# rwl/blu

Measured on AMD Instinct MI355X. Metric: factorize nnz/s + achieved HBM GB/s, 100k x 100k 10-nnz/col basis, higher is better.
Workload: dtype f64

## Files before the change

blu_amd/csrc/blu_dev.h:

```cpp
#pragma once
#include <hip/hip_runtime.h>
#include <stdint.h>
#include <hip/hip_cooperative_groups.h>
#include <rocprim/warp/warp_reduce.hpp>
#include <rocprim/warp/warp_scan.hpp>

#define BLU_WAVE 64

#ifndef BLU_DYN_SHARED
#define BLU_DYN_SHARED(T, name, bytes) extern __shared__ __attribute__((aligned(16))) T name[]
#endif
#ifdef BLU_PROFILE_FILLS
#define FILL_STAMP_BEGIN() long long fill_t0_ = (long long)__builtin_amdgcn_s_memtime()
#define FILL_STAMP(S, k)                                                 \
    do {                                                                 \
        if (threadIdx.x == 0) {                                          \
            const long long t_ = (long long)__builtin_amdgcn_s_memtime(); \
            (S)->prof[k] += t_ - fill_t0_;                               \
            fill_t0_ = t_;                                               \
        }                                                                \
    } while (0)
#else
#define FILL_STAMP_BEGIN() \
    do {                   \
    } while (0)
#define FILL_STAMP(S, k) \
    do {                 \
    } while (0)
#endif
#ifdef BLU_EMU_BUILD
#define BLU_WAVES_PER_EU(lo, hi)
#else
#define BLU_WAVES_PER_EU(lo, hi) __attribute__((amdgpu_waves_per_eu(lo, hi)))
#endif

enum {
    ST_RUNNING = 0,
    ST_DONE = 1,
    ST_STOPPED = 2,
    ST_NEED_L = 3,
    ST_NEED_U = 4,
    ST_NEED_CW = 5,
    ST_NEED_RW = 6,
    ST_INVALID_ARG = 7,
    ST_ERROR = 8
};

struct Scalars {
    int status;
    int err_line;
    int rank;
    int rankdef;
    int rank0;
    int min_colnz;
    int min_rownz;
    int pivot_row;
    int pivot_col;
    int bump_size;
    int cused, rused;
    int lused, uused;
    int need;
    int l_nz, u_nz;
    int fill_paths;
    long long matrix_nz;
    long long bump_nz;
    long long nsearch_pivot;
    long long factor_flops;
    long long nexpand;
    long long ngarbage;
    long long d3_hits;
    long long npivot_kind[6];
    long long nfast[4];
    double min_pivot, max_pivot;
    double onenorm, infnorm;
    double norm_l, norm_u, normest_l_inv, normest_u_inv, condest_l, condest_u, residual_test;
    long long prof[48];
};

#define DEVLU_SCALARS(X)                                                                               \
    X(int, m)                                                                                          \
    X(int, nzbias)                                                                      \
    X(int, maxsearch)                                                                                  \
    X(int, pad)                                                                                        \
    X(int, search_rows)                                                                                \
    X(int, no_fast)                    \
    X(int, skip_stats)              \
    X(double, droptol)                                                                                 \
    X(double, abstol)                                                                                  \
    X(double, reltol)                                                                                  \
    X(double, stretch)                                                                                 \
    X(long long, b_i_len)                                                                              \
    X(int, nzcap)                                                                                      \
    X(int, carena_cap)                                                                                 \
    X(int, rarena_cap)                                                                                 \
    X(int, lcap)                                                                                       \
    X(int, ucap)

#define DEVLU_ARRAYS_HOT(X)                                                                            \
    X(int, pinv) X(int, qinv) X(int, prow) X(int, pcol)                                                \
    X(LineRec, crec) X(LineRec, rrec) X(HeadRec, chead) X(HeadRec, rhead)                              \
    X(int, cidx) X(double, cval) X(int, ridx)                                                          \
    X(int, lbeg) X(int, ubeg) X(int, lidx) X(int, uidx) X(double, lval) X(double, uval)
#define DEVLU_ARRAYS_COLD(X)                                                                           \
    X(const unsigned long long, b_begin) X(const unsigned long long, b_end) X(const unsigned long long, b_i) \
    X(const double, b_x)                                                                               \
    X(int, bc_ptr) X(int, bc_idx) X(double, bc_val) X(int, bt_ptr) X(int, bt_idx) X(double, bt_val)    \
    X(int, rowmark) X(int, colmark) X(int, tnew) X(int, tnewr) X(double, txrj)                         \
    X(unsigned long long, tmask) X(double, gwork) X(int, iw0) X(int, iw1) X(int, iw2)
#define DEVLU_ARRAYS(X) DEVLU_ARRAYS_HOT(X) DEVLU_ARRAYS_COLD(X)

struct __attribute__((aligned(32))) LineRec {
    int beg, len, cap;
    int flink, blink;
    int spare;
    double max;
};
struct __attribute__((aligned(8))) HeadRec {
    int flink, blink;
};
static_assert(sizeof(LineRec) == 32 && sizeof(HeadRec) == 8, "record layout");
#define LINEREC_BEG 0
#define LINEREC_LEN 4
#define LINEREC_CAP 8
#define LINEREC_FLINK 12
#define LINEREC_BLINK 16
#define LINEREC_MAX 24

struct DevLU {
#define X(T, n) T n;
// ... 477 lines not shown
```

blu_amd/csrc/blu_hip.hip:

```cpp
#include <hip/hip_runtime.h>

#include <algorithm>
#include <cmath>
#include <cstdio>
#include <cstdlib>
#include <cstring>
#include <string>
#include <vector>

#include "../../include/blu_hip.h"
#include "blu_dev.h"
#include "k_finish.hip"
#define BLU_NS pv_single
#define BLU_CFG_WAVE 0
#include "k_pivot.hip"
#undef BLU_NS
#undef BLU_CFG_WAVE
#define BLU_NS pv_wave
#define BLU_CFG_WAVE 1
#include "k_pivot.hip"
#undef BLU_NS
#undef BLU_CFG_WAVE
#define BLU_NS pv_wave2
#define BLU_CFG_WAVE 2
// ... 436 lines not shown
    case BLU_STAT_NEXPAND: return (double)s.nexpand;
    case BLU_STAT_NGARBAGE: return (double)s.ngarbage;
    case BLU_STAT_FACTOR_FLOPS: return (double)s.factor_flops;
    case BLU_STAT_TIME_FACTORIZE: return h->t_total;
    case BLU_STAT_TIME_SINGLETONS: return h->t_phase[0];
    case BLU_STAT_TIME_SEARCH_PIVOT: {
        double tot = 0.0;
        for (int k = 0; k < 4; k++) tot += (double)s.prof[k];
        return tot > 0.0 ? h->t_pivot * (double)s.prof[0] / tot : 0.0;
    }
    case BLU_STAT_TIME_ELIM_PIVOT: {
        double tot = 0.0;
        for (int k = 0; k < 4; k++) tot += (double)s.prof[k];
        return tot > 0.0 ? h->t_pivot * (1.0 - (double)s.prof[0] / tot) : h->t_pivot;
    }
    case BLU_STAT_UPDATE_COST_DENOM: return h->update_cost_denom;
    case BLU_STAT_RANKDEF: return (double)s.rankdef;
    case BLU_STAT_L_MEM: return (double)h->D.lcap;
    case BLU_STAT_U_MEM: return (double)h->D.ucap;
    case BLU_STAT_W_MEM: return (double)h->D.carena_cap + (double)h->D.rarena_cap;
    case BLU_STAT_L_FLOPS: return (double)h->sp_l_flops;
    case BLU_STAT_U_FLOPS: return (double)h->sp_u_flops;
    case BLU_STAT_NFORREST: return h->upd_for_nfact == h->nfactorize ? (double)h->ust.nforrest : 0.0;
    case BLU_STAT_PIVOT_ERROR: return h->upd_for_nfact == h->nfactorize ? h->ust.pivot_error : 0.0;
    case BLU_STAT_R_NZ: return h->upd_for_nfact == h->nfactorize ? (double)h->ust.r_nz : 0.0;
    case BLU_STAT_R_FLOPS: return h->upd_for_nfact == h->nfactorize ? (double)h->ust.r_flops : 0.0;
    case BLU_STAT_MAX_ETA: return h->upd_for_nfact == h->nfactorize ? h->ust.max_eta : 0.0;
    case BLU_STAT_NSYMPERM_TOTAL: return (double)h->ust.nsymperm_total;
    case BLU_STAT_NFORREST_TOTAL: return (double)h->ust.nforrest_total;
    case BLU_STAT_DEV_NUNSYMPERM_TOTAL: return (double)h->ust.nunsymperm_total;
    case BLU_STAT_UPDATE_COST:
        return (h->upd_for_nfact == h->nfactorize ? h->ust.update_cost_numer : 0.0) / blu_hip_get_stat(h, BLU_STAT_UPDATE_COST_DENOM);
    case 44: case 45: case 46: case 47: return h->t_phase[key - 44];
    case 108: case 109: return h->t_phase[key - 108 + 4];
    case 43: return (double)h->sp_branch;
    case BLU_STAT_DEV_TIME_PIVOT_LOOP: return h->t_pivot;
    case BLU_STAT_DEV_TIME_TOTAL: return h->t_total;
    case BLU_STAT_DEV_RELAUNCHES: return (double)h->relaunches;
    case 50: return (double)s.d3_hits;
    case 51: return (double)s.npivot_kind[0];
    case 52: return (double)s.npivot_kind[1];
    case 53: return (double)s.npivot_kind[2];
    case 54: return (double)s.npivot_kind[3];
    case 55: return (double)s.npivot_kind[4];
    case 56: return (double)s.npivot_kind[5];
    case 110: case 111: case 116: case 117: return (double)s.nfast[key < 116 ? key - 110 : key - 114];
    case 112: return (double)s.cused;
    case 113: return (double)s.rused;
    case 114: return (double)h->D.carena_cap;
    case 115: return (double)h->D.lcap;
    case 120: return (double)h->last_pivot_regs;
    case 118: return (double)h->last_pivot_kernel;
    case 119: return (double)s.fill_paths;
    case 57: return (double)s.err_line;
    case 58: return (double)s.status;
    case 60: case 61: case 62: case 63: case 64: case 65: case 66: case 67: case 68: case 69: case 70: case 71: case 72: case 73: case 74: case 75:
    case 76: case 77: case 78: case 79: case 80: case 81: case 82: case 83:
    case 84: case 85: case 86: case 87: case 88: case 89: case 90: case 91:
    case 92: case 93: case 94: case 95: case 96: case 97: case 98: case 99: case 100: case 101: case 102: case 103: case 104: case 105: case 106: case 107:
        return (double)s.prof[key - 60];
    default: return NAN;
    }
}

extern "C" const char *blu_hip_last_error(const blu_hip *h) { return h ? h->err.c_str() : "null handle"; }
extern "C" const char *blu_hip_version(void)
{
#if defined(BLU_EWCHECK)
    return "blu_hip 0.2 (gfx950; self-checking build: early / speculative searches verified in the kernel)";
#elif defined(BLU_PROFILE)
    return "blu_hip 0.2 (gfx950; phase-timing build)";
#else
    return "blu_hip 0.2 (gfx950)";
#endif
}
extern "C" int blu_hip_device_count(void)
{
    int n = 0;
    if (hipGetDeviceCount(&n) != hipSuccess) return 0;
    return n;
}

static bool ensure_gwork(blu_hip *h, int cols)
{
    if (cols <= h->gwork_cols) return true;
    DevLU &D = h->D;
    const size_t n = (size_t)cols * ((size_t)h->m + 1);
    dfree(D.gwork);
    h->gwork_cols = 0;
    if (!dalloc(h, &D.gwork, n) || !hip_ok(h, hipMemset(D.gwork, 0, n * sizeof(double)), "hipMemset")) return false;
    h->gwork_cols = cols;
    return true;
}
static int64_t grown(blu_hip *h, int64_t cap, int64_t need_extra)
{
    const double f = std::max(1.0, h->realloc_factor);
    int64_t n = (int64_t)((double)(cap + need_extra) * f) + 64;
    return std::min<int64_t>(n, kIntMax);
}
static bool grow_l(blu_hip *h, int need)
{
    DevLU &D = h->D;
    const int64_t n = grown(h, D.lcap, need);
    if (n <= D.lcap) { h->err = "L storage limit (2^31 entries) reached"; return false; }
    if (!dgrow(h, &D.lidx, (size_t)h->hs.lused, (size_t)n) || !dgrow(h, &D.lval, (size_t)h->hs.lused, (size_t)n)) return false;
    D.lcap = (int)n;
// ... 594 lines not shown
```

blu_amd/csrc/k_pivot.hip:

```cpp
#include "blu_dev.h"

namespace BLU_NS {

__shared__ int g_pivot_err;
__shared__ int g_pivot_err_line;
#undef DEV_CHECK
#define DEV_CHECK(S, cond)                               \
    do {                                                 \
        if (!(cond)) {                                   \
            set_error((S), ST_ERROR, __LINE__);          \
            g_pivot_err = 1;                             \
        }                                                \
    } while (0)

#if BLU_CFG_WAVE
#include "k_pivot_wave_types.h"
#else
#include "k_pivot_fast_types.h"
#endif

#ifdef BLU_PROFILE
__shared__ long long g_pstamp[48];
#define PROF_STAMP(k)                                                      \
    do {                                                                   \
        if (threadIdx.x == 0) g_pstamp[k] = (long long)__builtin_amdgcn_s_memtime(); \
    } while (0)
#define PROF_STAMP_L0(k)                                                           \
    do {                                                                           \
        if (lane_id() == 0) g_pstamp[k] = (long long)__builtin_amdgcn_s_memtime(); \
    } while (0)
#define PROF_WAIT() asm volatile("s_waitcnt vmcnt(0)" ::: "memory")
#else
#define PROF_STAMP(k) \
    do {              \
    } while (0)
#define PROF_STAMP_L0(k) \
    do {                 \
    } while (0)
#define PROF_WAIT() \
    do {            \
    } while (0)
#endif

struct alignas(16) Sm {
    Fast fa;
    struct alignas(16) {
        int pr, pc, exit_code, head_exit;
    };
    struct alignas(16) {
        int nzc, nzr, pcb, prb;
    };
#ifdef BLU_PROFILE
    long long prof[48];
#else
    long long prof[1];
#endif
    int rank, rankdef, min_colnz, min_rownz;
    int cused, rused, lused, uused;
    int need;
    int flag_small;
    int other_row, where, ncancel, nfill;
    int stop_at, need_search;
    double pivot, other_value;
    long long nsearch, flops, nexpand, d3;
    long long kinds[6];
    long long nfast[4];
    int sh[40];
    long long shl[20];
#if BLU_CFG_WAVE
    unsigned long long wmax[BLU_CFG_WAVE];
#else
    unsigned long long wmax[16];
#endif
#if BLU_CFG_WAVE
    double swork[WV_WCAP];
#else
    double swork[16 * 64];
#endif
};

__device__ __forceinline__ void list_remove1(const LinkF &flink, const LinkB &blink, int e)
{
    const int f = flink[e], b = blink[e];
    flink[b] = f;
    blink[f] = b;
    flink[e] = e;
    blink[e] = e;
}
__device__ __forceinline__ void list_add1(int e, int list, const LinkF &flink, const LinkB &blink, int nelem)
{
    const int t = blink[nelem + list];
    blink[nelem + list] = e;
    blink[e] = t;
    flink[t] = e;
    flink[e] = nelem + list;
}

__device__ __forceinline__ int wave_list_move_batch(const LinkF &flink, const LinkB &blink, int nelem, gcint_p elems, gcint_p keys, int n,
                                                    gint_p mark, int big)
{
    const int lane = lane_id();
    int minkey = big;
    for (int c0 = 0; c0 < n; c0 += 64) {
        const int q = c0 + lane;
        if (q < n && keys[q] >= 0) mark[elems[q]] = 1;
    }
    wave_mem_sync();
    for (int c0 = 0; c0 < n; c0 += 64) {
// ... 980 lines not shown
    const int pr = sm->pr, pc = sm->pc;
    sm->fa.kind = 0;
    if (pc < 0 || pr < 0) return;
    sm->pcb = D.cbeg[pc];
    sm->prb = D.rbeg[pr];
    sm->nzc = D.clen[pc];
    sm->nzr = D.rlen[pr];
    sm->flag_small = 0;
    sm->ncancel = 0;
    DEV_CHECK(S, D.pinv[pr] == -1 && D.qinv[pc] == -1);
    DEV_CHECK(S, sm->nzc >= 1 && sm->nzr >= 1);
    if (sm->lused + (sm->nzc - 1) > D.lcap) {
        sm->exit_code = ST_NEED_L;
        sm->need = sm->nzc - 1;
    } else if (sm->uused + (sm->nzr - 1) > D.ucap) {
        sm->exit_code = ST_NEED_U;
        sm->need = sm->nzr - 1;
    }
}

#if BLU_CFG_WAVE
#include "k_pivot_wave.hip"
#else
__device__ __forceinline__ void pivot_loop_body(DevLU *Ds, int stop_at, Sm *sm, Mc *mc)
{
    const DevGP D(&Ds[blockIdx.x]);
    Scalars *S = D.s;
    const int tid = threadIdx.x, w = wave_id(), lane = lane_id();
    const int m = D.m;

    if (S->status != ST_RUNNING) return;
    if (tid == 0) {
        sm->rank = S->rank;
        sm->rankdef = S->rankdef;
        sm->min_colnz = S->min_colnz;
        sm->min_rownz = S->min_rownz;
        sm->cused = S->cused;
        sm->rused = S->rused;
        sm->lused = S->lused;
        sm->uused = S->uused;
        sm->pr = S->pivot_row;
        sm->pc = S->pivot_col;
        sm->exit_code = 0;
        sm->need = 0;
        sm->nsearch = 0;
        sm->flops = 0;
        sm->nexpand = 0;
        sm->d3 = 0;
        sm->stop_at = stop_at;
        sm->fa.kind = 0;
        sm->fa.ewValid = 0;
        sm->fa.spOk = 0;
        for (int k = 0; k < 6; k++) sm->kinds[k] = 0;
#ifdef BLU_PROFILE
        for (int k = 0; k < 48; k++) sm->prof[k] = 0;
        for (int k = 0; k < 48; k++) g_pstamp[k] = 0;
#endif
    }
    for (int k = tid; k < (int)blockDim.x; k += blockDim.x) sm->swork[k] = 0.0;
    if (tid < 16) sm->wmax[tid] = 0ull;
    for (int k = tid; k < 2 * KGMAX; k += blockDim.x) sm->fa.kg[0][k] = 0ull;
    if (tid == 0) {
        g_pivot_err = 0;
        g_pivot_err_line = 0;
    }
    mc_reset(D, mc, tid, (int)blockDim.x);
    __syncthreads();

    long long ew_mcb = 0;
    int ew_fb = 0;
    for (;;) {
        if (w == 0) {
            if (lane == 0) {
                if (g_pivot_err) sm->exit_code = ST_ERROR;
                else if (sm->rank + sm->rankdef >= m) sm->exit_code = ST_DONE;
                else if (sm->stop_at >= 0 && sm->pc < 0 && sm->rank + sm->rankdef >= sm->stop_at) sm->exit_code = ST_STOPPED;
                sm->need_search = sm->pc < 0;
                sm->head_exit = sm->exit_code;
            }
            wave_mem_sync();
            const bool heads_stale = mc->dirty;
            WAVE_LOCKSTEP();
            if (heads_stale) {
                mc_reset(D, mc, lane, 64);
                wave_mem_sync();
            }
            PROF_STAMP(0);
            if (!sm->head_exit) {
                bool handled = false;
                if (sm->need_search) {
                    if (D.search_rows == 0 && !D.no_fast) handled = markowitz_fast(D, sm, mc, ew_mcb, ew_fb);
                    if (!handled) {
                        if (D.search_rows == 0) markowitz_wave(D, sm);
                        else if (lane == 0) markowitz_serial(D, sm);
                        wave_mem_sync();
                    }
                }
                if (!handled && lane == 0) setup_pivot_general(D, sm);
            }
        }
        __syncthreads();
        const int4 dA = *reinterpret_cast<const int4 *>(&sm->pr);
        const int4 dB = *reinterpret_cast<const int4 *>(&sm->nzc);
        const int4 dC = *reinterpret_cast<const int4 *>(&sm->fa.kind);
        if (dA.w) break;
        const int pr = dA.x, pc = dA.y;
        if (pc < 0) {
            if (tid == 0) {
                DEV_CHECK(S, false);
                sm->exit_code = ST_ERROR;
            }
            __syncthreads();
            break;
        }
        if (pr < 0) {
            __syncthreads();
            if (tid == 0) {
                list_remove1(D.cflink, D.cblink, pc);
                mc->dirty = 1;
                sm->pc = -1;
                sm->rankdef++;
                sm->kinds[5]++;
            }
            __syncthreads();
            continue;
        }

        if (dA.z) break;
        PROF_STAMP(1);
        const int nz_col = dB.x, nz_row = dB.y;
        const int kind = dC.x;
        bool ok = true;
        if (kind == 1) fast_small(D, sm, mc, pr, pc, nz_col, nz_row, ew_mcb, ew_fb);
        else if (kind == 2) fast_scol(D, sm, mc, pr, pc, nz_row, dC.y, ew_mcb, ew_fb);
        else {
            if (tid == 0) mc->dirty = 1;
            if (nz_row == 1) ok = pivot_singleton_row(D, sm);
            else if (nz_col == 1) ok = pivot_singleton_col(D, sm);
            else if (nz_col == 2) ok = pivot_doubleton_col(D, sm);
            else ok = pivot_general(D, sm, nz_col - 1 <= 64);
        }
        if (!ok) break;
        PROF_STAMP(2);
#ifdef BLU_PROFILE
#define PROF_ADD(k, a, b)                                                                                           \
    do {                                                                                                            \
        const long long d_ = g_pstamp[a] - g_pstamp[b];                                                             \
        if (g_pstamp[b] >= g_pstamp[0] && d_ >= 0 && d_ < (1LL << 28)) sm->prof[k] += d_;                            \
    } while (0)
        if (tid == 0) {
            const int kk = sm->fa.kind == 1 ? 1 : (sm->fa.kind == 2 ? 2 : 3);
            PROF_ADD(0, 1, 0);
            PROF_ADD(kk, 2, 1);
            sm->prof[3 + kk] += 1;
            if (kk == 1) {
                PROF_ADD(7, 3, 1);
                PROF_ADD(22, 6, 3);
                PROF_ADD(23, 24, 3);
                PROF_ADD(24, 25, 3);
                PROF_ADD(25, 26, 25);
                PROF_ADD(26, 27, 26);
                PROF_ADD(27, 28, 27);
                PROF_ADD(30, 30, 27);
                PROF_ADD(31, 31, 30);
                PROF_ADD(28, 29, 28);
                PROF_ADD(29, 2, 29);
                sm->prof[32] += sm->nzr - 1;
                sm->prof[33] += sm->nzc - 1;
                PROF_ADD(34, 33, 1);
                PROF_ADD(35, 34, 33);
                PROF_ADD(36, 35, 34);
                PROF_ADD(37, 36, 35);
                PROF_ADD(38, 37, 36);
                PROF_ADD(39, 38, 37);
                PROF_ADD(40, 3, 38);
                if (g_pstamp[44] > g_pstamp[1]) {
                    PROF_ADD(41, 41, 1);
                    PROF_ADD(42, 42, 41);
                    PROF_ADD(43, 43, 42);
                    PROF_ADD(44, 44, 43);
                    sm->prof[45] += 1;
                }
            }
            if (kk != 3) {
                PROF_ADD(8, 8, 0);
                PROF_ADD(9, 9, 8);
                PROF_ADD(10, 10, 9);
                PROF_ADD(11, 11, 10);
                PROF_ADD(12, 12, 11);
                PROF_ADD(13, 13, 12);
                PROF_ADD(14, 14, 13);
                PROF_ADD(15, 1, 14);
                if (g_pstamp[16] > g_pstamp[8]) {
                    PROF_ADD(16, 17, 16);
                    PROF_ADD(17, 18, 17);
                    PROF_ADD(18, 10, 18);
                    PROF_ADD(19, 19, 8);
                    PROF_ADD(20, 20, 19);
                    sm->prof[21] += 1;
                }
            }
        }
#endif

        if (tid == 0) {
            const int rank = sm->rank;
            if (sm->flag_small && nz_row > 1) {
                for (int pos = D.ubeg[rank]; pos < D.ubeg[rank + 1]; pos++) {
                    const int j = D.uidx[pos];
                    if (D.colmax[j] == 0.0 || D.colmax[j] < D.abstol) {
                        remove_col_serial(D, sm, j);
                        mc->dirty = 1;
                    }
                }
            }
            sm->flops += (long long)(nz_col - 1) * (long long)(nz_row - 1);
            D.pinv[pr] = rank;
            D.qinv[pc] = rank;
            D.prow[rank] = pr;
            D.pcol[rank] = pc;
            sm->pc = -1;
            sm->pr = -1;
            sm->rank = rank + 1;
        }
    }

    if (tid == 0) {
        S->rank = sm->rank;
        S->rankdef = sm->rankdef;
        S->min_colnz = sm->min_colnz;
        S->min_rownz = sm->min_rownz;
        S->cused = sm->cused;
        S->rused = sm->rused;
        S->lused = sm->lused;
        S->uused = sm->uused;
        S->pivot_row = sm->pr;
        S->pivot_col = sm->pc;
        S->need = sm->need;
        S->nsearch_pivot += sm->nsearch;
        S->factor_flops += sm->flops;
        S->nexpand += sm->nexpand;
        S->d3_hits += sm->d3;
        for (int k = 0; k < 6; k++) S->npivot_kind[k] += sm->kinds[k];
#ifdef BLU_PROFILE
        for (int k = 0; k < 48; k++) S->prof[k] += sm->prof[k];
#endif
        if (sm->exit_code == ST_ERROR && g_pivot_err_line) set_error(S, ST_ERROR, g_pivot_err_line);
        if (S->status == ST_RUNNING) S->status = sm->exit_code;
    }
}

__global__ void __launch_bounds__(1024) k_pivot_loop(DevLU *Ds, int stop_at)
{
    __shared__ Sm smem;
    __shared__ Mc mcache;
    pivot_loop_body(Ds, stop_at, &smem, &mcache);
}
#endif

}
#undef PROF_STAMP
#undef PROF_STAMP_L0
#undef PROF_WAIT
#undef COLD
#undef DEV_CHECK
#define DEV_CHECK(S, cond)                                   \
    do {                                                     \
        if (!(cond)) set_error((S), ST_ERROR, __LINE__);     \
    } while (0)
```

blu_amd/csrc/k_pivot_fast.hip:

```cpp

__device__ __forceinline__ unsigned hslot(int k, int bits) { return ((unsigned)k * 2654435761u) >> (32 - bits); }
__device__ __forceinline__ void probe_overrun(int line)
{
    g_pivot_err = 1;
    g_pivot_err_line = line;
}
__device__ __forceinline__ void hrow_insert(Fast *f, int k, int v)
{
    unsigned s = hslot(k, HROW_BITS);
    const unsigned long long want = ((unsigned long long)(unsigned)k << 32) | (unsigned)v;
    for (int n = 0; n < HROW; n++) {
        const unsigned long long old = atomicCAS(&f->hRow[s], ~0ull, want);
        if (old == ~0ull || (int)(old >> 32) == k) return;
        s = (s + 1) & (HROW - 1);
    }
    probe_overrun(__LINE__);
}
__device__ __forceinline__ int hrow_lookup(const Fast *f, int k)
{
    unsigned s = hslot(k, HROW_BITS);
    for (int n = 0; n < HROW; n++) {
        const unsigned long long x = f->hRow[s];
        if ((int)(x >> 32) == k) return (int)(x & 0xffffffffull);
        if (x == ~0ull) return 0;
// ... 774 lines not shown
                const int n = hr_len[c] + nzr - 1;
                gr += n + stretch_of(D.stretch, n) + D.pad;
            }
        }
    }
#pragma unroll
    for (int c = 0; c < PRMAX / 64; c++) {
        const int q = c * 64 + lane;
        if (c * 64 < nzr && q < nzr) {
            const int j = jq[c];
            const int slot = kind == 1 ? ((q == wpos) ? 0 : (q == 0 ? wpos : q)) : q;
            const int tb = tbq[c], tl = tlq[c], tc = tcq[c];
            fa->tJ[slot] = j;
            fa->tB[slot] = tb;
            fa->tL[slot] = tl;
            fa->tC[slot] = tc;
            hcol_insert(fa, j, slot);
            if (kind == 1 && q != wpos) {
                const int n = tl + nzc - 1;
                gc += n + stretch_of(D.stretch, n) + D.pad;
            }
        }
    }
    PROF_STAMP(13);
    if (kind == 1) {
        const long long both = wave_sum_ll((gc << 32) | (gr & 0xffffffffLL));
        gc = both >> 32;
        gr = both & 0xffffffffLL;
        if ((long long)sm->cused + gc > (long long)D.carena_cap || (long long)sm->rused + gr > (long long)D.rarena_cap)
            kind = 0;
    }
    if (lane == 0) {
        fa->kind = kind;
        fa->where = wpos;
        fa->tLnk = 0;
    }
    PROF_STAMP(14);
}

__device__ __forceinline__ bool markowitz_fast(const DevGP &D, Sm *sm, Mc *mc, long long ew_mcb, int ew_fb)
{
    Fast *fa = &sm->fa;
    if (lane_id() == 0) fa->kind = 0;
    PROF_STAMP(8);
    int nsr = 0;
    if (fa->ewValid) {
        const int lane = lane_id();
        const bool whole = fa->ewValid == 2;
        const long long key = whole ? fa->spKey : -1;
        const long long mcb = ew_mcb;
        const int fb = ew_fb;
        nsr = fa->ewNsr;
        wave_mem_sync();
        if (lane == 0) fa->ewValid = 0;
#ifdef BLU_EWCHECK
        {
            const int sN = fa->ncand;
            const int myc = lane < sN ? fa->cJ[lane] : -1;
            const int sT = whole ? fa->cOff[sN] : 1;
            int kI[2], kB[2], kL[2], kC[2];
            double kV[2];
            for (int u = 0; u < 2; u++) {
                const int f = lane + 64 * u;
                kI[u] = f < sT ? fa->sI[f] : 0;
                kB[u] = f < sT ? fa->sB[f] : 0;
                kL[u] = f < sT ? fa->sL[f] : 0;
                kC[u] = f < sT ? fa->sC[f] : 0;
                kV[u] = f < sT ? fa->sV[f] : 0.0;
            }
            wave_mem_sync();
            int nsr2 = 0, fb2 = 0;
            long long mcb2 = 0;
            bool okc = true;
            if (whole || !mk_express(D, sm, mc, nsr2)) {
                const int r2 = mk_walk(D, sm, mc);
                if (r2 == 0) {
                    mk_stage(D, sm, mcb2, fb2);
                    nsr2 = fa->ncand;
                } else {
                    okc = false;
                }
            }
            if (whole) {
                const long long BIGK = 0x7fffffffffffffffLL;
                const long long key2 = wave_min_ll(mcb2 != BIGK ? mcb2 * 256LL + (long long)fb2 : BIGK);
                okc = okc && key2 == key && fa->cOff[fa->ncand] == sT;
                mcb2 = mcb;
                fb2 = fb;
            }
            for (int u = 0; u < 2; u++) {
                const int f = lane + 64 * u;
                if (okc && f < sT) okc = fa->sI[f] == kI[u] && fa->sB[f] == kB[u] && fa->sL[f] == kL[u] && fa->sC[f] == kC[u] && fa->sV[f] == kV[u];
            }
            okc = okc && fa->ncand == sN && nsr2 == nsr && mcb2 == mcb && fb2 == fb && (lane >= sN || fa->cJ[lane] == myc);
            if (__ballot(!okc)) {
                if (lane == 0 && D.s->prof[0] == 0) {
                    long long *P = D.s->prof;
                    P[0] = 1 + sm->rank;
                    P[1] = sN * 10 + fa->ncand;
                    P[2] = nsr * 10 + nsr2;
                    for (int i = 0; i < 3; i++) P[7 + i] = fa->cJ[i] * 1000LL + fa->cNz[i];
                }
                if (lane < 3) D.s->prof[10 + lane] = myc;
                DEV_CHECK(D.s, false);
            }
        }
#endif
// ... 327 lines not shown
    const int nk = __popcll(kb);
    const int need_max = nk + rnz1;
    const bool reloc = need_max > cap;
    int dst = rb, newcap = cap;
    if (reloc) {
        newcap = need_max + stretch_of(D.stretch, need_max) + D.pad;
        int nb = 0;
        if (lane == 0) nb = atomicAdd(&sm->rused, newcap);
        dst = __builtin_amdgcn_readfirstlane(nb);
    }
    if (keep) D.ridx[dst + t0] = j;
    for (int q = 1 + lane; q <= rnz1; q += 64) D.ridx[dst + nk + q - 1] = fa->tJ[q];
    if (lane == 0) {
        D.rbeg[i] = dst;
        D.rlen[i] = nk + rnz1;
        D.rcap[i] = newcap;
        fa->rNew[p] = nk + rnz1;
        fa->rKept[p] = nk;
        fa->rDst[p] = dst;
        if (reloc) atomicAdd((unsigned long long *)&sm->nexpand, 1ull);
    }
}

__device__ __forceinline__ void fast_fixrow(const DevGP &D, Sm *sm, int p)
{
    const int lane = lane_id();
    Fast *fa = &sm->fa;
    const int rnz1 = sm->nzr - 1;
    const int dst = fa->rDst[p], nk = fa->rKept[p];
    int na = 0;
    for (int c = 0; c < rnz1; c += 64) {
        const int q = 1 + c + lane;
        const bool ok = q <= rnz1 && ((fa->tM[q] >> (p - 1)) & 1ull) == 0;
        const unsigned long long kb = __ballot(ok);
        if (ok) D.ridx[dst + nk + na + wave_prefix_count(kb)] = fa->tJ[q];
        na += __popcll(kb);
    }
    if (lane == 0) {
        D.rlen[fa->pcI[p]] = nk + na;
        fa->rNew[p] = nk + na;
    }
}

__device__ __forceinline__ int wave_min_key(const int *keys, int n, int big)
{
    int v = big;
    for (int c = lane_id(); c < n; c += 64) {
        const int k = keys[c];
        if (k >= 0 && k < v) v = k;
    }
    return wave_min_i(v);
}

__device__ __forceinline__ void fast_write_u(const DevGP &D, Sm *sm, int q0, int q1, int skipq)
{
    const int lane = lane_id();
    Fast *fa = &sm->fa;
    int put = sm->uused;
    for (int c = q0; c <= q1; c += 64) {
        const int q = c + lane;
        const bool v = q <= q1 && q != skipq;
        const double x = v ? fa->tX[q] : 0.0;
        const bool k = v && fabs(x) > D.droptol;
        const unsigned long long kb = __ballot(k);
        if (k) {
            const int d = put + wave_prefix_count(kb);
            D.uidx[d] = fa->tJ[q];
            D.uval[d] = x;
        }
        put += __popcll(kb);
    }
    if (lane == 0) {
        D.ubeg[sm->rank + 1] = put;
        sm->uused = put;
    }
}

__device__ __forceinline__ void fast_write_l(const DevGP &D, Sm *sm)
{
    const int lane = lane_id();
    Fast *fa = &sm->fa;
    const int cnz1 = sm->nzc - 1;
    const double pivot = fa->pcV[0];
    int put = sm->lused;
    for (int c = 1; c <= cnz1; c += 64) {
        const int p = c + lane;
        const bool v = p <= cnz1;
        const double x = v ? fa->pcV[p] / pivot : 0.0;
        const bool k = v && fabs(x) > D.droptol;
        const unsigned long long kb = __ballot(k);
        if (k) {
            const int d = put + wave_prefix_count(kb);
            D.lidx[d] = fa->pcI[p];
            D.lval[d] = x;
        }
        put += __popcll(kb);
    }
    if (lane == 0) {
        D.lbeg[sm->rank + 1] = put;
        sm->lused = put;
    }
}

__device__ __forceinline__ void early_search(const DevGP &D, Sm *sm, Mc *mc, const int *elems, const int *keys, const int *begs, const double *maxs,
                                             int n, int ebase, long long &ew_mcb, int &ew_fb)
{
    const int lane = lane_id();
    const int m = D.m;
    Fast *fa = &sm->fa;
    const int K = D.maxsearch;
    if (D.search_rows || D.no_fast || K < 1 || K > KCMAX || m >= (1 << 27) || n >= 64) return;
    if (sm->flag_small || fa->anycancel) return;
    const int left = m - (sm->rank + 1) - sm->rankdef;
    if (left < 1) return;
    const int kq = lane < n ? keys[lane] : -1;
    if (__ballot(kq == 0)) return;
    int nsr = 0;

    {
        const int h1 = LinksC{D, mc}.fl(m + 1);
        const unsigned long long one = __ballot(kq == 1);
        int j = -1, cb = 0, fs = -1;
        double cmx = 0.0;
        if (h1 < m && !hcol_has(fa, h1)) {
            j = h1;
            cb = D.cbeg[j];
            cmx = D.colmax[j];
            if (D.clen[j] != 1) return;
        } else if (one) {
            const int l = __ffsll((long long)one) - 1;
            j = elems[l];
            cb = begs[l];
            cmx = maxs[l];
            if (ebase + l < MC_PREV && mc->e1i[ebase + l] >= 0 && mc->e1rl[ebase + l] >= 0) fs = ebase + l;
        }
        if (j >= 0) {
            if (cmx == 0.0 || !(cmx >= D.abstol)) return;
            int idx, rb, rl, rc;
            double val;
            if (fs >= 0) {
                idx = mc->e1i[fs];
                val = mc->e1v[fs];
                rb = mc->e1rb[fs];
                rl = mc->e1rl[fs];
                rc = mc->e1rc[fs];
            } else {
                idx = D.cidx[cb];
                val = D.cval[cb];
                rb = D.rbeg[idx];
                rl = D.rlen[idx];
                rc = D.rcap[idx];
            }
            const double tol = fmax(D.abstol, D.reltol * cmx);
            const double x = fabs(val);
            if (x == 0.0 || x < tol) return;
            nsr = left < K ? left : K;
            if (lane == 0) {
                fa->ncand = 1;
                fa->cJ[0] = j;
                fa->cNz[0] = 1;
                fa->cB[0] = cb;
                fa->cL[0] = 1;
                fa->cMx[0] = cmx;
                fa->cOff[0] = 0;
                fa->cOff[1] = 1;
                fa->sI[0] = idx;
                fa->sV[0] = val;
                fa->sB[0] = rb;
                fa->sL[0] = rl;
                fa->sC[0] = rc;
                fa->ewNsr = nsr;
                fa->ewValid = 1;
            }
            ew_mcb = 0;
            ew_fb = 0;
            wave_mem_sync();
            return;
// ... 224 lines not shown
            const int cb_ = fa->tB[q], cl_ = fa->tL[q], rb_ = fa->prB[p], rl_ = fa->prL[p];
            lb[u] = isc[u] ? cb_ : rb_;
            ll[u] = isc[u] ? cl_ : (isr ? rl_ : 0);
        }
#pragma unroll
        for (int u = 0; u < 3; u++) {
            li[u] = -1;
            lv[u] = 0.0;
            if (lane < ll[u]) {
                if (isc[u]) {
                    li[u] = D.cidx[lb[u] + lane];
                    lv[u] = D.cval[lb[u] + lane];
                } else {
                    li[u] = D.ridx[lb[u] + lane];
                }
            }
        }
#ifdef BLU_PROFILE
        if (w == 1 && base == 0) {
            PROF_STAMP_L0(33);
            PROF_WAIT();
            PROF_STAMP_L0(34);
        }
#endif
#pragma unroll
        for (int u = 0; u < 3; u++) {
            const int t = tt[u];
            if (t < rnz1) {
                if (ll[u] <= 64) fast_col_short(D, sm, mc, t + 1, work, li[u], lv[u], pr, cnz1, pivot);
                else fast_col(D, sm, mc, t + 1, work, li[u], lv[u], pr, cnz1, pivot);
            } else if (t < ntask) {
                if (ll[u] <= 64) fast_row_short(D, sm, t - rnz1 + 1, li[u], pc, rnz1);
                else fast_row(D, sm, t - rnz1 + 1, li[u], pc, rnz1);
            }
#ifdef BLU_PROFILE
            if (w == 1 && base == 0) PROF_STAMP_L0(35 + u);
#endif
        }
    }
#ifdef BLU_PROFILE
    if (w == 1) {
        PROF_WAIT();
        PROF_STAMP_L0(38);
    }
#endif
    PROF_STAMP(5);
    __syncthreads();
    PROF_STAMP(3);
    if (fa->anycancel) {
        for (int p = 1 + w; p <= cnz1; p += nw) fast_fixrow(D, sm, p);
        __syncthreads();
    }
    const bool spec = early && (w == 0 || w == nw - 1) && spec_cond(sm, fa->tNew + 1, rnz1);
    if (w == 0 && early && !spec) early_search(D, sm, mc, fa->tJ + 1, fa->tNew + 1, fa->tB + 1, fa->tMx + 1, rnz1, 1, ew_mcb, ew_fb);
    if (w == nw - 1 && spec) spec_finish(D, sm, rnz1);
    if (w == (early ? 3 : 0)) {
        fast_write_u(D, sm, 1, rnz1, -1);
        if (lane == 0) {
            D.colmax[pc] = fa->pcV[0];
            D.clen[pc] = 0;
            D.rlen[pr] = 0;
            sm->kinds[3]++;
        }
        PROF_STAMP_L0(6);
    }
    if (w == 1 % nw) {
        fast_write_l(D, sm);
        PROF_STAMP_L0(24);
    }
    if (w == 2 % nw) {
        PROF_STAMP_L0(25);
        const int mn = split ? wave_list_append_set(LC, m, fa->tJ + 1, fa->tNew + 1, rnz1, m + 2, fa->kg[0], mc->pFl + 1)
                             : wave_list_move_batch_set(LC, m, fa->tJ + 1, fa->tNew + 1, rnz1, InHCol{fa, 1, 0}, m + 2, pc, fa->kg[0]);
        if (lane == 0 && mn < sm->min_colnz) sm->min_colnz = mn;
        if (lane == 0) {
            mc->prevValid = split ? 1 : 0;
            mc->prevBase = 1;
        }
        PROF_WAIT();
        PROF_STAMP_L0(29);
    }
    if (D.search_rows && w == 3 % nw) {
        if (lane == 0) list_remove1(D.rflink, D.rblink, pr);
        wave_mem_sync();
        const int mn = wave_list_move_batch_set(LinksG{D.rflink, D.rblink}, m, fa->pcI + 1, fa->rNew + 1, cnz1, InHRow{fa}, m + 2, -1, fa->kg[1]);
        if (lane == 0 && mn < sm->min_rownz) sm->min_rownz = mn;
    }
    __syncthreads();
}

__device__ __forceinline__ void fast_scol(const DevGP &D, Sm *sm, Mc *mc, int pr, int pc, int rl, int wq, long long &ew_mcb, int &ew_fb)
{
    const int w = wave_id(), nw = num_waves(), lane = lane_id();
    const int m = D.m;
    Scalars *S = D.s;
    Fast *fa = &sm->fa;
    DEV_CHECK(S, fa->pcV[0] != 0.0 && fa->pcI[0] == pr);

    const bool split = nw >= 8 && rl < 64;
    const int nwt = split ? nw - 1 : nw;
    const LinksC LC{D, mc};
    if (split && w == nw - 1) {
        const bool lnk = fa->tLnk != 0;
        wave_list_unlink_set(LC, fa->tJ, rl, wq, InHCol{fa, 0, wq}, pc, lnk ? fa->tFl : nullptr, lnk ? fa->tBl : nullptr, wq);
    }
    for (int q = w; q < rl && w < nwt; q += nwt) {
        if (q == wq) {
            if (lane == 0) fa->tNew[q] = -1;
            continue;
        }
        const int j = fa->tJ[q], cb = fa->tB[q], cl = fa->tL[q];
        if (cl <= 64) {
            const bool v = lane < cl;
            const int idx = v ? D.cidx[cb + lane] : -1;
            const double val = v ? D.cval[cb + lane] : 0.0;
            const unsigned long long hb = __ballot(v && idx == pr);
            DEV_CHECK(S, hb != 0ull);
            const int src = hb ? __ffsll((long long)hb) - 1 : 0;
            const double xrj = wave_bcast_d(val, src);
            unsigned long long *wm = &sm->wmax[w];
            const bool fw1 = cl == 2 && q < MC_PREV && v && lane != src;
            int f_rb = 0, f_rl = 0, f_rc = 0;
            if (fw1) {
                f_rb = D.rbeg[idx];
                f_rl = D.rlen[idx];
                f_rc = D.rcap[idx];
                mc->e1i[q] = idx;
                mc->e1v[q] = val;
            }
            if (v && lane != src) {
                const double x = fabs(val);
                if (x > 0.0) atomicMax(wm, (unsigned long long)__double_as_longlong(x));
            }
            const int last_i = wave_bcast_i(idx, cl - 1);
            const double last_v = wave_bcast_d(val, cl - 1);
            wave_mem_sync();
            if (lane == 0 && hb) {
                const double cmx = __longlong_as_double((long long)*wm);
                *wm = 0ull;
                D.cidx[cb + src] = last_i;
                D.cval[cb + src] = last_v;
                D.clen[j] = cl - 1;
                D.colmax[j] = cmx;
                fa->tNew[q] = cl - 1;
                if (q < 64) fa->tMx[q] = cmx;
                if (cl != 2 && q < MC_PREV) mc->e1i[q] = -1;
                fa->tX[q] = xrj;
                if (cmx == 0.0 || cmx < D.abstol) sm->flag_small = 1;
            }
            if (fw1) {
                mc->e1rb[q] = f_rb;
                mc->e1rl[q] = f_rl;
                mc->e1rc[q] = f_rc;
            }
            continue;
        }
        int where = -1;
        double xrj = 0.0, cmxl = 0.0;
        for (int c = 0; c < cl; c += 64) {
            const int e = c + lane;
            const bool v = e < cl;
            const int idx = v ? D.cidx[cb + e] : -1;
            const double val = v ? D.cval[cb + e] : 0.0;
            const unsigned long long hb = __ballot(v && idx == pr);
            if (hb) {
                const int src = __ffsll((long long)hb) - 1;
                where = c + src;
                xrj = wave_bcast_d(val, src);
            }
            if (v && idx != pr) {
                const double x = fabs(val);
                if (x > cmxl) cmxl = x;
                if (cl == 2 && q < MC_PREV) {
                    mc->e1i[q] = idx;
                    mc->e1v[q] = val;
                    mc->e1rl[q] = -1;
                }
            }
        }
        DEV_CHECK(S, where >= 0);
        const double cmx = wave_max_d(cmxl);
        if (lane == 0 && where >= 0) {
            D.cidx[cb + where] = D.cidx[cb + cl - 1];
            D.cval[cb + where] = D.cval[cb + cl - 1];
            D.clen[j] = cl - 1;
            D.colmax[j] = cmx;
            fa->tNew[q] = cl - 1;
            if (q < 64) fa->tMx[q] = cmx;
            if (cl != 2 && q < MC_PREV) mc->e1i[q] = -1;
            fa->tX[q] = xrj;
            if (cmx == 0.0 || cmx < D.abstol) sm->flag_small = 1;
        }
    }
    __syncthreads();
    const bool early = split && !D.search_rows;
    if (w == 0 && early) early_search(D, sm, mc, fa->tJ, fa->tNew, fa->tB, fa->tMx, rl, 0, ew_mcb, ew_fb);
    if (w == (early ? 2 : 0)) {
        fast_write_u(D, sm, 0, rl - 1, wq);
        if (lane == 0) {
            D.lbeg[sm->rank + 1] = sm->lused;
            D.colmax[pc] = fa->pcV[0];
            D.clen[pc] = 0;
            D.rlen[pr] = 0;
            sm->kinds[1]++;
        }
    }
    if (w == 1 % nw) {
        if (D.search_rows && lane == 0) list_remove1(D.rflink, D.rblink, pr);
        const int mn = split ? wave_list_append_set(LC, m, fa->tJ, fa->tNew, rl, m + 2, fa->kg[0], mc->pFl)
                             : wave_list_move_batch_set(LC, m, fa->tJ, fa->tNew, rl, InHCol{fa, 0, wq}, m + 2, pc, fa->kg[0]);
        if (lane == 0 && mn < sm->min_colnz) sm->min_colnz = mn;
        if (lane == 0) {
            mc->prevValid = split ? 1 : 0;
            mc->prevBase = 0;
        }
    }
    __syncthreads();
}
```

Before: 1.319 million.

## Chain consecutive singleton-column pivots inside fast_scol using double-buffered Fast state

After the early search in fast_scol finds a valid next singleton-column pivot, the pivot setup (row index gather, hash insert) is done directly into a second Fast buffer. The loop then continues to the next pivot without going back through the main loop head, markowitz_fast and the extra block-wide barriers. The aim is to remove per-pivot search and synchronisation overhead on long runs of singleton-column pivots. The cost is a larger shared-memory footprint (a second Fast struct), extra bookkeeping and more complex control flow, along with some new profiling counters.

```diff
diff --git a/blu_amd/csrc/blu_dev.h b/blu_amd/csrc/blu_dev.h
--- a/blu_amd/csrc/blu_dev.h
+++ b/blu_amd/csrc/blu_dev.h
@@ -71,10 +71,12 @@
     long long d3_hits;
     long long npivot_kind[6];
     long long nfast[4];
+    long long nrun[2];
     double min_pivot, max_pivot;
     double onenorm, infnorm;
     double norm_l, norm_u, normest_l_inv, normest_u_inv, condest_l, condest_u, residual_test;
     long long prof[48];
+    long long prof2[8];
 };
 
 #define DEVLU_SCALARS(X)                                                                               \
diff --git a/blu_amd/csrc/blu_hip.hip b/blu_amd/csrc/blu_hip.hip
--- a/blu_amd/csrc/blu_hip.hip
+++ b/blu_amd/csrc/blu_hip.hip
@@ -512,6 +512,8 @@
     case 120: return (double)h->last_pivot_regs;
     case 118: return (double)h->last_pivot_kernel;
     case 119: return (double)s.fill_paths;
+    case 121: case 122: return (double)s.nrun[key - 121];
+    case 131: case 132: case 133: case 134: case 135: case 136: case 137: case 138: return (double)s.prof2[key - 131];
     case 57: return (double)s.err_line;
     case 58: return (double)s.status;
     case 60: case 61: case 62: case 63: case 64: case 65: case 66: case 67: case 68: case 69: case 70: case 71: case 72: case 73: case 74: case 75:
diff --git a/blu_amd/csrc/k_pivot.hip b/blu_amd/csrc/k_pivot.hip
--- a/blu_amd/csrc/k_pivot.hip
+++ b/blu_amd/csrc/k_pivot.hip
@@ -20,7 +20,7 @@
 #endif
 
 #ifdef BLU_PROFILE
-__shared__ long long g_pstamp[48];
+__shared__ long long g_pstamp[56];
 #define PROF_STAMP(k)                                                      \
     do {                                                                   \
         if (threadIdx.x == 0) g_pstamp[k] = (long long)__builtin_amdgcn_s_memtime(); \
@@ -52,8 +52,18 @@
     };
 #ifdef BLU_PROFILE
     long long prof[48];
+    long long prof2[8];
 #else
     long long prof[1];
+#endif
+#if !BLU_CFG_WAVE
+    Fast fb;
+    struct alignas(16) {
+        int nx_pr, nx_pc, nx_nzr, nx_where;
+    };
+    int nx_prb, nx_pcb, nx_nsr;
+    int mg;
+    long long nrun[2];
 #endif
     int rank, rankdef, min_colnz, min_rownz;
     int cused, rused, lused, uused;
@@ -1140,9 +1150,12 @@
         sm->fa.ewValid = 0;
         sm->fa.spOk = 0;
         for (int k = 0; k < 6; k++) sm->kinds[k] = 0;
+        sm->mg = 0;
+        sm->nrun[0] = sm->nrun[1] = 0;
 #ifdef BLU_PROFILE
         for (int k = 0; k < 48; k++) sm->prof[k] = 0;
-        for (int k = 0; k < 48; k++) g_pstamp[k] = 0;
+        for (int k = 0; k < 8; k++) sm->prof2[k] = 0;
+        for (int k = 0; k < 56; k++) g_pstamp[k] = 0;
 #endif
     }
     for (int k = tid; k < (int)blockDim.x; k += blockDim.x) sm->swork[k] = 0.0;
@@ -1155,89 +1168,20 @@
     mc_reset(D, mc, tid, (int)blockDim.x);
     __syncthreads();
 
-    long long ew_mcb = 0;
-    int ew_fb = 0;
-    for (;;) {
-        if (w == 0) {
-            if (lane == 0) {
-                if (g_pivot_err) sm->exit_code = ST_ERROR;
-                else if (sm->rank + sm->rankdef >= m) sm->exit_code = ST_DONE;
-                else if (sm->stop_at >= 0 && sm->pc < 0 && sm->rank + sm->rankdef >= sm->stop_at) sm->exit_code = ST_STOPPED;
-                sm->need_search = sm->pc < 0;
-                sm->head_exit = sm->exit_code;
-            }
-            wave_mem_sync();
-            const bool heads_stale = mc->dirty;
-            WAVE_LOCKSTEP();
-            if (heads_stale) {
-                mc_reset(D, mc, lane, 64);
-                wave_mem_sync();
-            }
-            PROF_STAMP(0);
-            if (!sm->head_exit) {
-                bool handled = false;
-                if (sm->need_search) {
-                    if (D.search_rows == 0 && !D.no_fast) handled = markowitz_fast(D, sm, mc, ew_mcb, ew_fb);
-                    if (!handled) {
-                        if (D.search_rows == 0) markowitz_wave(D, sm);
-                        else if (lane == 0) markowitz_serial(D, sm);
-                        wave_mem_sync();
-                    }
-                }
-                if (!handled && lane == 0) setup_pivot_general(D, sm);
-            }
-        }
-        __syncthreads();
-        const int4 dA = *reinterpret_cast<const int4 *>(&sm->pr);
-        const int4 dB = *reinterpret_cast<const int4 *>(&sm->nzc);
-        const int4 dC = *reinterpret_cast<const int4 *>(&sm->fa.kind);
-        if (dA.w) break;
-        const int pr = dA.x, pc = dA.y;
-        if (pc < 0) {
-            if (tid == 0) {
-                DEV_CHECK(S, false);
-                sm->exit_code = ST_ERROR;
-            }
-            __syncthreads();
-            break;
-        }
-        if (pr < 0) {
-            __syncthreads();
-            if (tid == 0) {
-                list_remove1(D.cflink, D.cblink, pc);
-                mc->dirty = 1;
-                sm->pc = -1;
-                sm->rankdef++;
-                sm->kinds[5]++;
-            }
-            __syncthreads();
-            continue;
-        }
-
-        if (dA.z) break;
-        PROF_STAMP(1);
-        const int nz_col = dB.x, nz_row = dB.y;
-        const int kind = dC.x;
-        bool ok = true;
-        if (kind == 1) fast_small(D, sm, mc, pr, pc, nz_col, nz_row, ew_mcb, ew_fb);
-        else if (kind == 2) fast_scol(D, sm, mc, pr, pc, nz_row, dC.y, ew_mcb, ew_fb);
-        else {
-            if (tid == 0) mc->dirty = 1;
-            if (nz_row == 1) ok = pivot_singleton_row(D, sm);
-            else if (nz_col == 1) ok = pivot_singleton_col(D, sm);
-            else if (nz_col == 2) ok = pivot_doubleton_col(D, sm);
-            else ok = pivot_general(D, sm, nz_col - 1 <= 64);
-        }
-        if (!ok) break;
-        PROF_STAMP(2);
 #ifdef BLU_PROFILE
 #define PROF_ADD(k, a, b)                                                                                           \
     do {                                                                                                            \
         const long long d_ = g_pstamp[a] - g_pstamp[b];                                                             \
         if (g_pstamp[b] >= g_pstamp[0] && d_ >= 0 && d_ < (1LL << 28)) sm->prof[k] += d_;                            \
     } while (0)
-        if (tid == 0) {
-            const int kk = sm->fa.kind == 1 ? 1 : (sm->fa.kind == 2 ? 2 : 3);
+#define PROF_ADD2(k, a, b)                                                                                          \
+    do {                                                                                                            \
+        const long long d_ = g_pstamp[a] - g_pstamp[b];                                                             \
+        if (g_pstamp[b] >= g_pstamp[0] && d_ >= 0 && d_ < (1LL << 28)) sm->prof2[k] += d_;                           \
+    } while (0)
+    auto prof_account = [&](int kind_done) {
+        {
+            const int kk = kind_done == 1 ? 1 : (kind_done == 2 ? 2 : 3);
             PROF_ADD(0, 1, 0);
             PROF_ADD(kk, 2, 1);
             sm->prof[3 + kk] += 1;
@@ -1270,6 +1214,14 @@
                     sm->prof[45] += 1;
                 }
             }
+            if (kk == 2) {
+                PROF_ADD2(0, 1, 0);
+                PROF_ADD2(1, 49, 48);
+                PROF_ADD2(2, 50, 48);
+                PROF_ADD2(3, 51, 48);
+                PROF_ADD2(4, 2, 48);
+                PROF_ADD2(5, 48, 1);
+            }
             if (kk != 3) {
                 PROF_ADD(8, 8, 0);
                 PROF_ADD(9, 9, 8);
@@ -1289,6 +1241,123 @@
                 }
             }
         }
+    };
+#endif
+    long long ew_mcb = 0;
+    int ew_fb = 0;
+    for (;;) {
+        if (w == 0) {
+            if (lane == 0) {
+                if (g_pivot_err) sm->exit_code = ST_ERROR;
+                else if (sm->rank + sm->rankdef >= m) sm->exit_code = ST_DONE;
+                else if (sm->stop_at >= 0 && sm->pc < 0 && sm->rank + sm->rankdef >= sm->stop_at) sm->exit_code = ST_STOPPED;
+                sm->need_search = sm->pc < 0;
+                sm->head_exit = sm->exit_code;
+            }
+            wave_mem_sync();
+            const bool heads_stale = mc->dirty;
+            WAVE_LOCKSTEP();
+            if (heads_stale) {
+                mc_reset(D, mc, lane, 64);
+                wave_mem_sync();
+            }
+            PROF_STAMP(0);
+            if (!sm->head_exit) {
+                bool handled = false;
+                if (sm->need_search) {
+                    if (D.search_rows == 0 && !D.no_fast) handled = markowitz_fast(D, sm, mc, ew_mcb, ew_fb);
+                    if (!handled) {
+                        if (D.search_rows == 0) markowitz_wave(D, sm);
+                        else if (lane == 0) markowitz_serial(D, sm);
+                        wave_mem_sync();
+                    }
+                }
+                if (!handled && lane == 0) setup_pivot_general(D, sm);
+            }
+        }
+        __syncthreads();
+        const int4 dA = *reinterpret_cast<const int4 *>(&sm->pr);
+        const int4 dB = *reinterpret_cast<const int4 *>(&sm->nzc);
+        const int4 dC = *reinterpret_cast<const int4 *>(&sm->fa.kind);
+        if (dA.w) break;
+        int pr = dA.x, pc = dA.y;
+        if (pc < 0) {
+            if (tid == 0) {
+                DEV_CHECK(S, false);
+                sm->exit_code = ST_ERROR;
+            }
+            __syncthreads();
+            break;
+        }
+        if (pr < 0) {
+            __syncthreads();
+            if (tid == 0) {
+                list_remove1(D.cflink, D.cblink, pc);
+                mc->dirty = 1;
+                sm->pc = -1;
+                sm->rankdef++;
+                sm->kinds[5]++;
+            }
+            __syncthreads();
+            continue;
+        }
+
+        if (dA.z) break;
+        PROF_STAMP(1);
+        const int nz_col = dB.x;
+        int nz_row = dB.y;
+        const int kind = dC.x;
+        bool ok = true;
+        if (kind == 1) fast_small(D, sm, mc, pr, pc, nz_col, nz_row, ew_mcb, ew_fb);
+        else if (kind == 2) {
+            Fast *cs = &sm->fa;
+            int wq = dC.y;
+            for (;;) {
+                fast_scol(D, sm, mc, cs, pr, pc, nz_row, wq, ew_mcb, ew_fb);
+                if (!sm->mg) break;
+#ifdef BLU_PROFILE
+                PROF_STAMP(2);
+                if (tid == 0) {
+                    prof_account(2);
+                    sm->prof2[6] += 1;
+                    g_pstamp[0] = g_pstamp[1] = g_pstamp[2];
+                }
+#endif
+                const int4 nx = *reinterpret_cast<const int4 *>(&sm->nx_pr);
+                if (tid == (int)blockDim.x - 128) {
+                    const int rank = sm->rank;
+                    D.pinv[pr] = rank;
+                    D.qinv[pc] = rank;
+                    D.prow[rank] = pr;
+                    D.pcol[rank] = pc;
+                    sm->rank = rank + 1;
+                    sm->nsearch += sm->nx_nsr;
+                    sm->min_colnz = 1;
+                    sm->nrun[0]++;
+                    sm->nrun[1]++;
+                }
+                pr = nx.x;
+                pc = nx.y;
+                nz_row = nx.z;
+                wq = nx.w;
+                cs = cs == &sm->fa ? &sm->fb : &sm->fa;
+#ifdef BLU_EWCHECK
+                __syncthreads();
+                if (w == 0) scol_setup_check(D, sm, mc, cs);
+                __syncthreads();
+#endif
+            }
+        } else {
+            if (tid == 0) mc->dirty = 1;
+            if (nz_row == 1) ok = pivot_singleton_row(D, sm);
+            else if (nz_col == 1) ok = pivot_singleton_col(D, sm);
+            else if (nz_col == 2) ok = pivot_doubleton_col(D, sm);
+            else ok = pivot_general(D, sm, nz_col - 1 <= 64);
+        }
+        if (!ok) break;
+        PROF_STAMP(2);
+#ifdef BLU_PROFILE
+        if (tid == 0) prof_account(kind);
 #endif
 
         if (tid == 0) {
@@ -1330,8 +1399,10 @@
         S->nexpand += sm->nexpand;
         S->d3_hits += sm->d3;
         for (int k = 0; k < 6; k++) S->npivot_kind[k] += sm->kinds[k];
+        for (int k = 0; k < 2; k++) S->nrun[k] += sm->nrun[k];
 #ifdef BLU_PROFILE
         for (int k = 0; k < 48; k++) S->prof[k] += sm->prof[k];
+        for (int k = 0; k < 8; k++) S->prof2[k] += sm->prof2[k];
 #endif
         if (sm->exit_code == ST_ERROR && g_pivot_err_line) set_error(S, ST_ERROR, g_pivot_err_line);
         if (S->status == ST_RUNNING) S->status = sm->exit_code;
diff --git a/blu_amd/csrc/k_pivot_fast.hip b/blu_amd/csrc/k_pivot_fast.hip
--- a/blu_amd/csrc/k_pivot_fast.hip
+++ b/blu_amd/csrc/k_pivot_fast.hip
@@ -850,7 +850,10 @@
         const int fb = ew_fb;
         nsr = fa->ewNsr;
         wave_mem_sync();
-        if (lane == 0) fa->ewValid = 0;
+        if (lane == 0) {
+            if (!whole) sm->nrun[0]++;
+            fa->ewValid = 0;
+        }
 #ifdef BLU_EWCHECK
         {
             const int sN = fa->ncand;
@@ -1284,10 +1287,9 @@
     return wave_min_i(v);
 }
 
-__device__ __forceinline__ void fast_write_u(const DevGP &D, Sm *sm, int q0, int q1, int skipq)
+__device__ __forceinline__ void fast_write_u(const DevGP &D, Sm *sm, const Fast *fa, int q0, int q1, int skipq)
 {
     const int lane = lane_id();
-    Fast *fa = &sm->fa;
     int put = sm->uused;
     for (int c = q0; c <= q1; c += 64) {
         const int q = c + lane;
@@ -1334,7 +1336,7 @@
     }
 }
 
-__device__ __forceinline__ void early_search(const DevGP &D, Sm *sm, Mc *mc, const int *elems, const int *keys, const int *begs, const double *maxs,
+__device__ __forceinline__ void early_search(const DevGP &D, Sm *sm, Mc *mc, const Fast *cs, const int *elems, const int *keys, const int *begs, const double *maxs,
                                              int n, int ebase, long long &ew_mcb, int &ew_fb)
 {
     const int lane = lane_id();
@@ -1354,7 +1356,7 @@
         const unsigned long long one = __ballot(kq == 1);
         int j = -1, cb = 0, fs = -1;
         double cmx = 0.0;
-        if (h1 < m && !hcol_has(fa, h1)) {
+        if (h1 < m && !hcol_has(cs, h1)) {
             j = h1;
             cb = D.cbeg[j];
             cmx = D.colmax[j];
@@ -1685,10 +1687,10 @@
         __syncthreads();
     }
     const bool spec = early && (w == 0 || w == nw - 1) && spec_cond(sm, fa->tNew + 1, rnz1);
-    if (w == 0 && early && !spec) early_search(D, sm, mc, fa->tJ + 1, fa->tNew + 1, fa->tB + 1, fa->tMx + 1, rnz1, 1, ew_mcb, ew_fb);
+    if (w == 0 && early && !spec) early_search(D, sm, mc, fa, fa->tJ + 1, fa->tNew + 1, fa->tB + 1, fa->tMx + 1, rnz1, 1, ew_mcb, ew_fb);
     if (w == nw - 1 && spec) spec_finish(D, sm, rnz1);
     if (w == (early ? 3 : 0)) {
-        fast_write_u(D, sm, 1, rnz1, -1);
+        fast_write_u(D, sm, fa, 1, rnz1, -1);
         if (lane == 0) {
             D.colmax[pc] = fa->pcV[0];
             D.clen[pc] = 0;
@@ -1722,12 +1724,120 @@
     __syncthreads();
 }
 
-__device__ __forceinline__ void fast_scol(const DevGP &D, Sm *sm, Mc *mc, int pr, int pc, int rl, int wq, long long &ew_mcb, int &ew_fb)
+__device__ __forceinline__ bool scol_setup_next(const DevGP &D, Sm *sm, Mc *mc, Fast *nxt, int rl_cur)
+{
+    const int lane = lane_id();
+    Fast *st = &sm->fa;
+    if (st->ewValid != 1) return false;
+    if (g_pivot_err || mc->dirty) return false;
+    const int nrd = sm->rank + 1 + sm->rankdef;
+    if (nrd >= D.m || (sm->stop_at >= 0 && nrd >= sm->stop_at)) return false;
+    const int pc = st->cJ[0], pr = st->sI[0], prb = st->sB[0], nzr = st->sL[0];
+    if (nzr < 2 || nzr >= 64) return false;
+    if (sm->lused > D.lcap || (long long)sm->uused + (rl_cur - 1) + (nzr - 1) > (long long)D.ucap) return false;
+    const int jq0 = lane < nzr ? D.ridx[prb + lane] : -1;
+    for (int s = lane; s < HCOL; s += 64) nxt->hCol[s] = ~0ull;
+    const unsigned long long hb = __ballot(jq0 == pc);
+    if (!hb) return false;
+    const int wpos = __ffsll((long long)hb) - 1;
+    if (lane < nzr) {
+        const int tb = D.cbeg[jq0], tl = D.clen[jq0], tc = D.ccap[jq0];
+        nxt->tJ[lane] = jq0;
+        nxt->tB[lane] = tb;
+        nxt->tL[lane] = tl;
+        nxt->tC[lane] = tc;
+        hcol_insert(nxt, jq0, lane);
+    }
+    if (lane == 0) {
+        nxt->pcI[0] = pr;
+        nxt->pcV[0] = st->sV[0];
+        nxt->prB[0] = prb;
+        nxt->prL[0] = nzr;
+        nxt->prC[0] = st->sC[0];
+        nxt->kind = 2;
+        nxt->where = wpos;
+        nxt->tLnk = 0;
+        sm->nx_pr = pr;
+        sm->nx_pc = pc;
+        sm->nx_nzr = nzr;
+        sm->nx_where = wpos;
+        sm->nx_prb = prb;
+        sm->nx_pcb = st->cB[0];
+        sm->nx_nsr = st->ewNsr;
+        st->ewValid = 0;
+    }
+    return true;
+}
+
+#ifdef BLU_EWCHECK
+__device__ __forceinline__ void scol_setup_check(const DevGP &D, Sm *sm, Mc *mc, Fast *nxt)
+{
+    const int lane = lane_id();
+    Fast *T = nxt;
+    Fast *R = &sm->fa;
+    if (nxt == R) {
+        T = &sm->fb;
+        T->tJ[lane] = R->tJ[lane];
+        T->tB[lane] = R->tB[lane];
+        T->tL[lane] = R->tL[lane];
+        T->tC[lane] = R->tC[lane];
+        for (int s = lane; s < HCOL; s += 64) T->hCol[s] = R->hCol[s];
+        if (lane == 0) {
+            T->kind = R->kind;
+            T->where = R->where;
+            T->pcI[0] = R->pcI[0];
+            T->pcV[0] = R->pcV[0];
+        }
+    }
+    wave_mem_sync();
+    const int o_pr = sm->pr, o_pc = sm->pc, o_pcb = sm->pcb, o_prb = sm->prb, o_nzc = sm->nzc, o_nzr = sm->nzr;
+    const int o_exit = sm->exit_code, o_need = sm->need, o_minc = sm->min_colnz;
+    const long long o_ns = sm->nsearch;
+    wave_mem_sync();
+    int nsr2 = 0;
+    bool okc = mk_express(D, sm, mc, nsr2);
+    if (okc) {
+        mk_pick(D, sm, 0, 0, nsr2, true);
+        wave_mem_sync();
+        const int n = sm->nx_nzr;
+        okc = sm->pr == sm->nx_pr && sm->pc == sm->nx_pc && sm->nzr == n && sm->nzc == 1 && sm->prb == sm->nx_prb && sm->pcb == sm->nx_pcb &&
+              nsr2 == sm->nx_nsr && sm->exit_code == o_exit && sm->min_colnz == o_minc && R->kind == 2 && T->kind == 2 && R->where == T->where &&
+              R->pcI[0] == T->pcI[0] && R->pcV[0] == T->pcV[0];
+        if (okc && lane < n) {
+            const int j = T->tJ[lane];
+            okc = R->tJ[lane] == j && R->tB[lane] == T->tB[lane] && R->tL[lane] == T->tL[lane] && R->tC[lane] == T->tC[lane] &&
+                  hcol_slot(R, j) == lane && hcol_slot(T, j) == lane;
+        }
+        int cntR = 0, cntT = 0;
+        for (int s = lane; s < HCOL; s += 64) {
+            cntR += __popcll(__ballot(R->hCol[s] != ~0ull));
+            cntT += __popcll(__ballot(T->hCol[s] != ~0ull));
+        }
+        okc = okc && cntR == n && cntT == n;
+    }
+    wave_mem_sync();
+    if (lane == 0) {
+        sm->pr = o_pr;
+        sm->pc = o_pc;
+        sm->pcb = o_pcb;
+        sm->prb = o_prb;
+        sm->nzc = o_nzc;
+        sm->nzr = o_nzr;
+        sm->exit_code = o_exit;
+        sm->need = o_need;
+        sm->min_colnz = o_minc;
+        sm->nsearch = o_ns;
+    }
+    if (__ballot(!okc)) DEV_CHECK(D.s, false);
+    wave_mem_sync();
+}
+#endif
+
+__device__ __forceinline__ void fast_scol(const DevGP &D, Sm *sm, Mc *mc, Fast *fa, int pr, int pc, int rl, int wq, long long &ew_mcb, int &ew_fb)
 {
     const int w = wave_id(), nw = num_waves(), lane = lane_id();
     const int m = D.m;
     Scalars *S = D.s;
-    Fast *fa = &sm->fa;
     DEV_CHECK(S, fa->pcV[0] != 0.0 && fa->pcI[0] == pr);
 
     const bool split = nw >= 8 && rl < 64;
@@ -1827,9 +1937,18 @@
     }
     __syncthreads();
     const bool early = split && !D.search_rows;
-    if (w == 0 && early) early_search(D, sm, mc, fa->tJ, fa->tNew, fa->tB, fa->tMx, rl, 0, ew_mcb, ew_fb);
+    PROF_STAMP(48);
+    if (w == 0) {
+        bool merged = false;
+        if (early) {
+            early_search(D, sm, mc, fa, fa->tJ, fa->tNew, fa->tB, fa->tMx, rl, 0, ew_mcb, ew_fb);
+            merged = scol_setup_next(D, sm, mc, fa == &sm->fa ? &sm->fb : &sm->fa, rl);
+        }
+        if (lane == 0) sm->mg = merged ? 1 : 0;
+        PROF_STAMP(49);
+    }
     if (w == (early ? 2 : 0)) {
-        fast_write_u(D, sm, 0, rl - 1, wq);
+        fast_write_u(D, sm, fa, 0, rl - 1, wq);
         if (lane == 0) {
             D.lbeg[sm->rank + 1] = sm->lused;
             D.colmax[pc] = fa->pcV[0];
@@ -1837,16 +1956,18 @@
             D.rlen[pr] = 0;
             sm->kinds[1]++;
         }
+        if (w != 0) PROF_STAMP_L0(50);
     }
     if (w == 1 % nw) {
         if (D.search_rows && lane == 0) list_remove1(D.rflink, D.rblink, pr);
-        const int mn = split ? wave_list_append_set(LC, m, fa->tJ, fa->tNew, rl, m + 2, fa->kg[0], mc->pFl)
-                             : wave_list_move_batch_set(LC, m, fa->tJ, fa->tNew, rl, InHCol{fa, 0, wq}, m + 2, pc, fa->kg[0]);
+        const int mn = split ? wave_list_append_set(LC, m, fa->tJ, fa->tNew, rl, m + 2, sm->fa.kg[0], mc->pFl)
+                             : wave_list_move_batch_set(LC, m, fa->tJ, fa->tNew, rl, InHCol{fa, 0, wq}, m + 2, pc, sm->fa.kg[0]);
         if (lane == 0 && mn < sm->min_colnz) sm->min_colnz = mn;
         if (lane == 0) {
-            mc->prevValid = split ? 1 : 0;
+            mc->prevValid = split && fa == &sm->fa ? 1 : 0;
             mc->prevBase = 0;
         }
+        if (w != 0) PROF_STAMP_L0(51);
     }
     __syncthreads();
 }
```

New measurement: 1.378 million (median of 6 runs). 1.04x the previous value.
